# stanfordnlp/mac-network

Measured on NVIDIA H100. Metric: mac_reasoning_steps_per_sec, higher is better.
Workload: dtype bf16

## Files before the change

mac_network_b200/csrc/read_step.cuh:

```cuda
#pragma once
#include "tc_gemm.cuh"

namespace mac {

constexpr int RS_D = 512;
constexpr int RS_BM = 64;
constexpr int RS_KB = RS_D / TC_BK;
constexpr int RS_BLK = RS_BM * TC_BK * 2;
constexpr int RS_A_BYTES = RS_KB * RS_BLK;
constexpr int RS_B_HALF = 256 * TC_BK * 2;
constexpr int RS_CONSUMERS = 256;
constexpr int RS_THREADS = RS_CONSUMERS + 32;

constexpr int RS128_BM = 128;
constexpr int RS128_BLK = RS128_BM * TC_BK * 2;
constexpr int RS128_A_BYTES = RS_KB * RS128_BLK;
constexpr int RS128_STAGE = RS_B_HALF;
constexpr int RS128_STAGES = 3;
constexpr int RS128_Q0 = RS_KB;
constexpr int RS128_G1B = RS128_Q0 + 2;
constexpr int RS128_Q1 = RS128_G1B + RS_KB;
constexpr int RS128_G2A = RS128_Q1 + 2;
constexpr int RS128_G2B = RS128_G2A + RS_KB;
constexpr int RS128_SLOTS = RS128_G2B + RS_KB;
constexpr int RS128_CONSUMERS = 256;
constexpr int RS128_THREADS = RS128_CONSUMERS + 128;
constexpr int RS128_SMEM_BYTES = RS128_A_BYTES + RS128_STAGES * RS128_STAGE + 1024  +
                                 8 * (RS_KB + 2 * RS128_STAGES) ;
static_assert(RS128_SMEM_BYTES <= 232448, "over the sm_90 per-block shared memory opt-in limit");
static_assert(RS128_BLK % 1024 == 0 && RS128_STAGE % 1024 == 0 && (RS128_BM / 2) * 128 % 1024 == 0,
              "swizzled operands need 1024-byte alignment");
static_assert(2 * RS128_BLK == RS128_STAGE, "a ring slot holds two Q blocks");
constexpr int RS128_PRODUCER_REGS = 40;
constexpr int RS128_CONSUMER_REGS = 232;
static_assert(RS128_PRODUCER_REGS + 2 * RS128_CONSUMER_REGS <= 3 * (65536 / RS128_THREADS / 8 * 8), "register budget");

__device__ __forceinline__ float bf16lo(uint32_t w) { return __uint_as_float(w << 16); }
__device__ __forceinline__ float bf16hi(uint32_t w) { return __uint_as_float(w & 0xffff0000u); }

__device__ __forceinline__ void wgmma_bf16_n256(float (&d)[128], uint64_t adesc, uint64_t bdesc, uint32_t accum) {
  asm volatile(
      "{\n\t.reg .pred p;\n\t"
      "setp.ne.b32 p, %130, 0;\n\t"
      "wgmma.mma_async.sync.aligned.m64n256k16.f32.bf16.bf16 "
      "{%0, %1, %2, %3, %4, %5, %6, %7, %8, %9, %10, %11, %12, %13, %14, %15, %16, %17, %18, %19, %20, %21, %22, %23, %24, %25, %26, %27, %28, %29, %30, %31, %32, %33, %34, %35, %36, %37, %38, %39, %40, %41, %42, %43, %44, %45, %46, %47, %48, %49, %50, %51, %52, %53, %54, %55, %56, %57, %58, %59, %60, %61, %62, %63, %64, %65, %66, %67, %68, %69, %70, %71, %72, %73, %74, %75, %76, %77, %78, %79, %80, %81, %82, %83, %84, %85, %86, %87, %88, %89, %90, %91, %92, %93, %94, %95, %96, %97, %98, %99, %100, %101, %102, %103, %104, %105, %106, %107, %108, %109, %110, %111, %112, %113, %114, %115, %116, %117, %118, %119, %120, %121, %122, %123, %124, %125, %126, %127}, %128, %129, p, 1, 1, 0, 0;\n\t}"
      : "+f"(d[0]), "+f"(d[1]), "+f"(d[2]), "+f"(d[3]), "+f"(d[4]), "+f"(d[5]), "+f"(d[6]), "+f"(d[7]), "+f"(d[8]), "+f"(d[9]), "+f"(d[10]), "+f"(d[11]), "+f"(d[12]), "+f"(d[13]), "+f"(d[14]), "+f"(d[15]), "+f"(d[16]), "+f"(d[17]), "+f"(d[18]), "+f"(d[19]), "+f"(d[20]), "+f"(d[21]), "+f"(d[22]), "+f"(d[23]), "+f"(d[24]), "+f"(d[25]), "+f"(d[26]), "+f"(d[27]), "+f"(d[28]), "+f"(d[29]), "+f"(d[30]), "+f"(d[31]), "+f"(d[32]), "+f"(d[33]), "+f"(d[34]), "+f"(d[35]), "+f"(d[36]), "+f"(d[37]), "+f"(d[38]), "+f"(d[39]), "+f"(d[40]), "+f"(d[41]), "+f"(d[42]), "+f"(d[43]), "+f"(d[44]), "+f"(d[45]), "+f"(d[46]), "+f"(d[47]), "+f"(d[48]), "+f"(d[49]), "+f"(d[50]), "+f"(d[51]), "+f"(d[52]), "+f"(d[53]), "+f"(d[54]), "+f"(d[55]), "+f"(d[56]), "+f"(d[57]), "+f"(d[58]), "+f"(d[59]), "+f"(d[60]), "+f"(d[61]), "+f"(d[62]), "+f"(d[63]), "+f"(d[64]), "+f"(d[65]), "+f"(d[66]), "+f"(d[67]), "+f"(d[68]), "+f"(d[69]), "+f"(d[70]), "+f"(d[71]), "+f"(d[72]), "+f"(d[73]), "+f"(d[74]), "+f"(d[75]), "+f"(d[76]), "+f"(d[77]), "+f"(d[78]), "+f"(d[79]), "+f"(d[80]), "+f"(d[81]), "+f"(d[82]), "+f"(d[83]), "+f"(d[84]), "+f"(d[85]), "+f"(d[86]), "+f"(d[87]), "+f"(d[88]), "+f"(d[89]), "+f"(d[90]), "+f"(d[91]), "+f"(d[92]), "+f"(d[93]), "+f"(d[94]), "+f"(d[95]), "+f"(d[96]), "+f"(d[97]), "+f"(d[98]), "+f"(d[99]), "+f"(d[100]), "+f"(d[101]), "+f"(d[102]), "+f"(d[103]), "+f"(d[104]), "+f"(d[105]), "+f"(d[106]), "+f"(d[107]), "+f"(d[108]), "+f"(d[109]), "+f"(d[110]), "+f"(d[111]), "+f"(d[112]), "+f"(d[113]), "+f"(d[114]), "+f"(d[115]), "+f"(d[116]), "+f"(d[117]), "+f"(d[118]), "+f"(d[119]), "+f"(d[120]), "+f"(d[121]), "+f"(d[122]), "+f"(d[123]), "+f"(d[124]), "+f"(d[125]), "+f"(d[126]), "+f"(d[127])
      : "l"(adesc), "l"(bdesc), "r"(accum));
}
inline bool read_step_supported(int B, int N, int d) {
  return d == RS_D && N >= 1 && N <= 256 && B >= 1 && B < (1 << 22);
}

struct ReadStepParams {
  int M, N;
  const float* y;
  const float* ctrl;
  const float* bm2;
  const float* wr;
  float* logits;
};

__device__ __forceinline__ void rs_consumer_bar() { asm volatile("bar.sync 1, %0;" ::"n"(RS_CONSUMERS) : "memory"); }

__device__ __forceinline__ void rs128_wg_bar(int g) { asm volatile("bar.sync %0, 128;" ::"r"(1 + g) : "memory"); }

__device__ __forceinline__ void rs128_gemm_half(float (&acc)[128], uint32_t a_u, uint32_t ring_u, uint64_t* full,
                                                uint64_t* empty, int t0, int lane) {
  for (int j = 0; j < RS_KB; ++j) {
    const int t = t0 + j, s = t % RS128_STAGES;
    mbar_wait(&full[s], (t / RS128_STAGES) & 1);
    const uint64_t adesc = make_sw128_kmajor_desc(a_u + j * RS128_BLK);
    const uint64_t bdesc = make_sw128_kmajor_desc(ring_u + s * RS128_STAGE);
    wgmma_fence();
#pragma unroll
    for (int k = 0; k < TC_BK / 16; ++k) wgmma_bf16_n256(acc, adesc + 2 * k, bdesc + 2 * k, (j || k) ? 1u : 0u);
    wgmma_commit();
    wgmma_wait<1>();
    wgmma_hold(acc);
    if (j && lane == 0) mbar_arrive(&empty[(t - 1) % RS128_STAGES]);
  }
  wgmma_wait<0>();
  wgmma_hold(acc);
  if (lane == 0) mbar_arrive(&empty[(t0 + RS_KB - 1) % RS128_STAGES]);
}

__device__ __forceinline__ int rs128_sw_off(int r, int n, int blk) {
  return (n >> 6) * blk + r * 128 + ((((n & 63) >> 3) ^ (r & 7)) << 4) + (n & 7) * 2;
}

__global__ void __launch_bounds__(RS128_THREADS, 1)
read_step_kernel(const __grid_constant__ CUtensorMap map_p, const __grid_constant__ CUtensorMap map_q,
                 const __grid_constant__ CUtensorMap map_w1, const __grid_constant__ CUtensorMap map_w2,
                 const ReadStepParams p) {
  extern __shared__ unsigned char smem_dyn[];
  const uint32_t base_u32 = smem_u32(smem_dyn);
  unsigned char* a_tile = smem_dyn + ((1024u - (base_u32 & 1023u)) & 1023u);
  unsigned char* ring = a_tile + RS128_A_BYTES;
  uint64_t* pfull = reinterpret_cast<uint64_t*>(ring + RS128_STAGES * RS128_STAGE);
  uint64_t* full = pfull + RS_KB;
  uint64_t* empty = full + RS128_STAGES;

  const int warp = threadIdx.x >> 5, lane = threadIdx.x & 31;
  const int row0 = blockIdx.x * RS128_BM;

  if (threadIdx.x == RS128_CONSUMERS) {
    tma_prefetch_desc(&map_p);
    tma_prefetch_desc(&map_q);
    tma_prefetch_desc(&map_w1);
    tma_prefetch_desc(&map_w2);
    for (int i = 0; i < RS_KB; ++i) mbar_init(&pfull[i], 1);
    for (int i = 0; i < RS128_STAGES; ++i) {
      mbar_init(&full[i], 1);
      mbar_init(&empty[i], RS128_CONSUMERS / 32);
    }
    fence_mbar_init();
  }
  __syncthreads();

  if (warp >= RS128_CONSUMERS / 32) {
    asm volatile("setmaxnreg.dec.sync.aligned.u32 %0;" ::"n"(RS128_PRODUCER_REGS));
    if (warp == RS128_CONSUMERS / 32 && elect_one()) {
      auto load_p = [&](int j) {
        mbar_expect_tx(&pfull[j], RS128_BLK);
        tma_load_2d(a_tile + j * RS128_BLK, &map_p, j * TC_BK, row0, &pfull[j]);
      };
      for (int t = 0; t < RS128_SLOTS; ++t) {
        if (t < RS128_STAGES) load_p(t);
        else if (t == RS128_STAGES)
          for (int j = RS128_STAGES; j < RS_KB; ++j) load_p(j);
        const int s = t % RS128_STAGES;
        mbar_wait(&empty[s], ((t / RS128_STAGES) & 1) ^ 1);
        unsigned char* dst = ring + s * RS128_STAGE;
        mbar_expect_tx(&full[s], RS128_STAGE);
        if (t < RS128_G2A) {
          const int half = t >= RS128_G1B, u = t - half * RS128_G1B;
          if (u < RS_KB) {
            tma_load_2d(dst, &map_w1, u * TC_BK, 256 * half, &full[s]);
          } else {
            const int kb = 4 * half + 2 * (u - RS_KB);
            tma_load_2d(dst, &map_q, kb * TC_BK, row0, &full[s]);
            tma_load_2d(dst + RS128_BLK, &map_q, (kb + 1) * TC_BK, row0, &full[s]);
          }
        } else {
          const int half = t >= RS128_G2B, u = t - (half ? RS128_G2B : RS128_G2A);
          tma_load_2d(dst, &map_w2, u * TC_BK, 256 * half, &full[s]);
        }
      }
    }
    return;
  }

  asm volatile("setmaxnreg.inc.sync.aligned.u32 %0;" ::"n"(RS128_CONSUMER_REGS));
  const int g = warp >> 2;
  const int wt = threadIdx.x & 127;
  const int rl = 16 * (warp & 3) + (lane >> 2);
  const int cq = 2 * (lane & 3);
  const int rowg = row0 + 64 * g;
  unsigned char* a_wg = a_tile + g * (RS128_BM / 2) * 128;
  const uint32_t a_u = smem_u32(a_wg), ring_u = smem_u32(ring);
  const int prow = wt >> 3;
  const int poff = prow * 128 + (wt & 7) * 16;
  const int pcol = ((wt & 7) ^ (prow & 7)) << 3;
  int yoff[4];
#pragma unroll
  for (int u = 0; u < 4; ++u) yoff[u] = min(rowg + prow + 16 * u, p.M - 1) / p.N * RS_D + pcol;

  float acc[128];
  float4 y0[4], y1[4];
  auto load_y = [&](int j) {
#pragma unroll
    for (int u = 0; u < 4; ++u) {
      y0[u] = *reinterpret_cast<const float4*>(p.y + yoff[u] + j * TC_BK);
      y1[u] = *reinterpret_cast<const float4*>(p.y + yoff[u] + j * TC_BK + 4);
    }
  };
  load_y(0);
  for (int j = 0; j < RS_KB; ++j) {
    const int s = j % RS128_STAGES;
    mbar_wait(&pfull[j], 0);
#pragma unroll
    for (int u = 0; u < 4; ++u) {
      uint4* c = reinterpret_cast<uint4*>(a_wg + j * RS128_BLK + poff + u * 16 * 128);
      const uint4 v = *c;
      *c = make_uint4(pack_bf16(bf16lo(v.x) * y0[u].x, bf16hi(v.x) * y0[u].y), pack_bf16(bf16lo(v.y) * y0[u].z, bf16hi(v.y) * y0[u].w),
                      pack_bf16(bf16lo(v.z) * y1[u].x, bf16hi(v.z) * y1[u].y), pack_bf16(bf16lo(v.w) * y1[u].z, bf16hi(v.w) * y1[u].w));
    }
    fence_proxy_async();
    rs128_wg_bar(g);
    mbar_wait(&full[s], (j / RS128_STAGES) & 1);
    const uint64_t adesc = make_sw128_kmajor_desc(a_u + j * RS128_BLK);
    const uint64_t bdesc = make_sw128_kmajor_desc(ring_u + s * RS128_STAGE);
    wgmma_fence();
#pragma unroll
    for (int k = 0; k < TC_BK / 16; ++k) wgmma_bf16_n256(acc, adesc + 2 * k, bdesc + 2 * k, (j || k) ? 1u : 0u);
    wgmma_commit();
    if (j + 1 < RS_KB) load_y(j + 1);
    wgmma_wait<1>();
    wgmma_hold(acc);
    if (j && lane == 0) mbar_arrive(&empty[(j - 1) % RS128_STAGES]);
  }
  wgmma_wait<0>();
  wgmma_hold(acc);
  if (lane == 0) mbar_arrive(&empty[(RS_KB - 1) % RS128_STAGES]);

  uint32_t h0[64];
#pragma unroll
  for (int q = 0; q < 2; ++q) {
    const int t = RS128_Q0 + q, s = t % RS128_STAGES;
    mbar_wait(&full[s], (t / RS128_STAGES) & 1);
    const unsigned char* q_tile = ring + s * RS128_STAGE + g * (RS128_BM / 2) * 128 - 2 * q * RS128_BLK;
#pragma unroll
    for (int h = 0; h < 2; ++h) {
      const int r = rl + 8 * h;
      const bool live = rowg + r < p.M;
#pragma unroll
      for (int j = 16 * q; j < 16 * q + 16; ++j) {
        const uint32_t qv = *reinterpret_cast<const uint32_t*>(q_tile + rs128_sw_off(r, cq + 8 * j, RS128_BLK));
        h0[2 * j + h] = live ? pack_bf16(elu_fast(acc[4 * j + 2 * h] + bf16lo(qv)), elu_fast(acc[4 * j + 2 * h + 1] + bf16hi(qv)))
                             : 0u;
      }
    }
    __syncwarp();
    if (lane == 0) mbar_arrive(&empty[s]);
  }

  rs128_gemm_half(acc, a_u, ring_u, full, empty, RS128_G1B, lane);

  rs128_wg_bar(g);
#pragma unroll
  for (int h = 0; h < 2; ++h) {
    const int r = rl + 8 * h;
#pragma unroll
    for (int j = 0; j < 32; ++j) *reinterpret_cast<uint32_t*>(a_wg + rs128_sw_off(r, cq + 8 * j, RS128_BLK)) = h0[2 * j + h];
  }
#pragma unroll
  for (int q = 0; q < 2; ++q) {
    const int t = RS128_Q1 + q, s = t % RS128_STAGES;
    mbar_wait(&full[s], (t / RS128_STAGES) & 1);
    const unsigned char* q_tile = ring + s * RS128_STAGE + g * (RS128_BM / 2) * 128 - 2 * q * RS128_BLK;
#pragma unroll
    for (int h = 0; h < 2; ++h) {
      const int r = rl + 8 * h;
      const bool live = rowg + r < p.M;
#pragma unroll
      for (int j = 16 * q; j < 16 * q + 16; ++j) {
        const int n = cq + 8 * j;
        const uint32_t qv = *reinterpret_cast<const uint32_t*>(q_tile + rs128_sw_off(r, n, RS128_BLK));
        *reinterpret_cast<uint32_t*>(a_wg + rs128_sw_off(r, 256 + n, RS128_BLK)) =
            live ? pack_bf16(elu_fast(acc[4 * j + 2 * h] + bf16lo(qv)), elu_fast(acc[4 * j + 2 * h + 1] + bf16hi(qv))) : 0u;
      }
    }
    __syncwarp();
    if (lane == 0) mbar_arrive(&empty[s]);
  }
  fence_proxy_async();
  rs128_wg_bar(g);

  float part[2][2];
#pragma unroll
  for (int half = 0; half < 2; ++half) {
    rs128_gemm_half(acc, a_u, ring_u, full, empty, half ? RS128_G2B : RS128_G2A, lane);
#pragma unroll
    for (int h = 0; h < 2; ++h) {
      const int row = rowg + rl + 8 * h;
      const float* crow = p.ctrl + (size_t)(min(row, p.M - 1) / p.N) * RS_D + 256 * half;
      const float* bm2 = p.bm2 + 256 * half;
      const float* wr = p.wr + 256 * half;
      float s = 0.f;
#pragma unroll
      for (int j = 0; j < 32; ++j) {
        const int n = cq + 8 * j;
        const float2 cc = __ldg(reinterpret_cast<const float2*>(crow + n));
        const float2 bb = __ldg(reinterpret_cast<const float2*>(bm2 + n));
        const float2 ww = __ldg(reinterpret_cast<const float2*>(wr + n));
        const float t0 = elu_fast((acc[4 * j + 2 * h] + bb.x) * cc.x);
        const float t1 = elu_fast((acc[4 * j + 2 * h + 1] + bb.y) * cc.y);
        s = fmaf(t0, ww.x, s);
        s = fmaf(t1, ww.y, s);
      }
      s += __shfl_xor_sync(0xffffffffu, s, 1);
      s += __shfl_xor_sync(0xffffffffu, s, 2);
      part[half][h] = s;
    }
  }
#pragma unroll
  for (int h = 0; h < 2; ++h) {
    const int row = rowg + rl + 8 * h;
    if ((lane & 3) == 0 && row < p.M) p.logits[row] = part[0][h] + part[1][h];
  }
}

inline int read_step_launch(const void* P, const void* Q, float* logits, const void* kb_bf16, const float* y,
                            const float* control, const mac_read_weights* w, float* att, float* info, int B, int N, int d,
                            cudaStream_t stream) {
  const int M = B * N;
  CUtensorMap mp, mq, mw1, mw2;
  int st = make_tmap_2d(&mp, P, 1, (uint64_t)M, (uint64_t)d, (uint64_t)d * 2, RS128_BM, TC_BK, 1);
  if (st != MAC_OK) return st;
  st = make_tmap_2d(&mq, Q, 1, (uint64_t)M, (uint64_t)d, (uint64_t)d * 2, RS128_BM, TC_BK, 1);
  if (st != MAC_OK) return st;
  st = make_tmap_2d(&mw1, w->Wm_bf16, 1, (uint64_t)d, (uint64_t)d, (uint64_t)2 * d * 2, 256, TC_BK, 1);
  if (st != MAC_OK) return st;
  st = make_tmap_2d(&mw2, w->Wm2_bf16, 1, (uint64_t)d, (uint64_t)d, (uint64_t)d * 2, 256, TC_BK, 1);
  if (st != MAC_OK) return st;
  ReadStepParams p{};
  p.M = M; p.N = N; p.y = y; p.ctrl = control; p.bm2 = w->bm2; p.wr = w->wr; p.logits = logits;
  MAC_CUDA_TRY(cudaFuncSetAttribute(read_step_kernel, cudaFuncAttributeMaxDynamicSharedMemorySize, RS128_SMEM_BYTES));
  read_step_kernel<<<(M + RS128_BM - 1) / RS128_BM, RS128_THREADS, RS128_SMEM_BYTES, stream>>>(mp, mq, mw1, mw2, p);
  MAC_LAUNCH_CHECK();
  return mac_kb_attend_fwd(logits, 1, w->br, kb_bf16, 1, att, info, B, N, d, stream);
}

}
```

Baseline: 21560.

## Feed GEMM1 A operand from registers via ldmatrix and stream P with weights

GEMM 1 no longer loads P fully into shared memory, scales it by y in place and issues an SS wgmma. P tiles are now streamed through a two-stage ring alongside the W1 tiles, loaded into registers with ldmatrix, scaled by y in registers, and fed to register-sourced wgmma. This removes the shared-memory write-back, the async-proxy fence and the warpgroup barrier on each k-block. Q is loaded directly into the A tile, so the h epilogue updates it in place instead of staging it through the ring and a 64-register h0 buffer. The trade-off is higher register pressure from the A fragments and y values, plus a more complex barrier layout.

```diff
diff --git a/mac_network_b200/csrc/read_step.cuh b/mac_network_b200/csrc/read_step.cuh
--- a/mac_network_b200/csrc/read_step.cuh
+++ b/mac_network_b200/csrc/read_step.cuh
@@ -17,20 +17,21 @@
 constexpr int RS128_A_BYTES = RS_KB * RS128_BLK;
 constexpr int RS128_STAGE = RS_B_HALF;
 constexpr int RS128_STAGES = 3;
-constexpr int RS128_Q0 = RS_KB;
-constexpr int RS128_G1B = RS128_Q0 + 2;
-constexpr int RS128_Q1 = RS128_G1B + RS_KB;
-constexpr int RS128_G2A = RS128_Q1 + 2;
-constexpr int RS128_G2B = RS128_G2A + RS_KB;
-constexpr int RS128_SLOTS = RS128_G2B + RS_KB;
+constexpr int RS128_RING_BYTES = RS128_STAGES * RS128_STAGE;
 constexpr int RS128_CONSUMERS = 256;
 constexpr int RS128_THREADS = RS128_CONSUMERS + 128;
-constexpr int RS128_SMEM_BYTES = RS128_A_BYTES + RS128_STAGES * RS128_STAGE + 1024  +
+constexpr int RS128_SMEM_BYTES = RS128_A_BYTES + RS128_RING_BYTES + 1024  +
                                  8 * (RS_KB + 2 * RS128_STAGES) ;
 static_assert(RS128_SMEM_BYTES <= 232448, "over the sm_90 per-block shared memory opt-in limit");
 static_assert(RS128_BLK % 1024 == 0 && RS128_STAGE % 1024 == 0 && (RS128_BM / 2) * 128 % 1024 == 0,
               "swizzled operands need 1024-byte alignment");
-static_assert(2 * RS128_BLK == RS128_STAGE, "a ring slot holds two Q blocks");
+constexpr int RS128_P_STAGE = RS_B_HALF + RS128_BLK;
+constexpr int RS128_P_STAGES = 2;
+constexpr int RS128_G1_SLOTS = 2 * RS_KB;
+static_assert(RS128_P_STAGES * RS128_P_STAGE <= RS128_RING_BYTES && RS128_P_STAGE % 1024 == 0, "GEMM 1 ring");
+constexpr int RS128_STEP_SMEM_BYTES = RS128_A_BYTES + RS128_RING_BYTES + 1024  +
+                                      8 * (RS_KB + 2 * RS128_P_STAGES + 2 * RS128_STAGES) ;
+static_assert(RS128_STEP_SMEM_BYTES <= 232448, "over the sm_90 per-block shared memory opt-in limit");
 constexpr int RS128_PRODUCER_REGS = 40;
 constexpr int RS128_CONSUMER_REGS = 232;
 static_assert(RS128_PRODUCER_REGS + 2 * RS128_CONSUMER_REGS <= 3 * (65536 / RS128_THREADS / 8 * 8), "register budget");
@@ -47,6 +48,19 @@
       : "+f"(d[0]), "+f"(d[1]), "+f"(d[2]), "+f"(d[3]), "+f"(d[4]), "+f"(d[5]), "+f"(d[6]), "+f"(d[7]), "+f"(d[8]), "+f"(d[9]), "+f"(d[10]), "+f"(d[11]), "+f"(d[12]), "+f"(d[13]), "+f"(d[14]), "+f"(d[15]), "+f"(d[16]), "+f"(d[17]), "+f"(d[18]), "+f"(d[19]), "+f"(d[20]), "+f"(d[21]), "+f"(d[22]), "+f"(d[23]), "+f"(d[24]), "+f"(d[25]), "+f"(d[26]), "+f"(d[27]), "+f"(d[28]), "+f"(d[29]), "+f"(d[30]), "+f"(d[31]), "+f"(d[32]), "+f"(d[33]), "+f"(d[34]), "+f"(d[35]), "+f"(d[36]), "+f"(d[37]), "+f"(d[38]), "+f"(d[39]), "+f"(d[40]), "+f"(d[41]), "+f"(d[42]), "+f"(d[43]), "+f"(d[44]), "+f"(d[45]), "+f"(d[46]), "+f"(d[47]), "+f"(d[48]), "+f"(d[49]), "+f"(d[50]), "+f"(d[51]), "+f"(d[52]), "+f"(d[53]), "+f"(d[54]), "+f"(d[55]), "+f"(d[56]), "+f"(d[57]), "+f"(d[58]), "+f"(d[59]), "+f"(d[60]), "+f"(d[61]), "+f"(d[62]), "+f"(d[63]), "+f"(d[64]), "+f"(d[65]), "+f"(d[66]), "+f"(d[67]), "+f"(d[68]), "+f"(d[69]), "+f"(d[70]), "+f"(d[71]), "+f"(d[72]), "+f"(d[73]), "+f"(d[74]), "+f"(d[75]), "+f"(d[76]), "+f"(d[77]), "+f"(d[78]), "+f"(d[79]), "+f"(d[80]), "+f"(d[81]), "+f"(d[82]), "+f"(d[83]), "+f"(d[84]), "+f"(d[85]), "+f"(d[86]), "+f"(d[87]), "+f"(d[88]), "+f"(d[89]), "+f"(d[90]), "+f"(d[91]), "+f"(d[92]), "+f"(d[93]), "+f"(d[94]), "+f"(d[95]), "+f"(d[96]), "+f"(d[97]), "+f"(d[98]), "+f"(d[99]), "+f"(d[100]), "+f"(d[101]), "+f"(d[102]), "+f"(d[103]), "+f"(d[104]), "+f"(d[105]), "+f"(d[106]), "+f"(d[107]), "+f"(d[108]), "+f"(d[109]), "+f"(d[110]), "+f"(d[111]), "+f"(d[112]), "+f"(d[113]), "+f"(d[114]), "+f"(d[115]), "+f"(d[116]), "+f"(d[117]), "+f"(d[118]), "+f"(d[119]), "+f"(d[120]), "+f"(d[121]), "+f"(d[122]), "+f"(d[123]), "+f"(d[124]), "+f"(d[125]), "+f"(d[126]), "+f"(d[127])
       : "l"(adesc), "l"(bdesc), "r"(accum));
 }
+__device__ __forceinline__ void wgmma_bf16_n256_rs(float (&d)[128], const uint32_t (&a)[4], uint64_t bdesc, uint32_t accum) {
+  asm volatile(
+      "{\n\t.reg .pred p;\n\t"
+      "setp.ne.b32 p, %133, 0;\n\t"
+      "wgmma.mma_async.sync.aligned.m64n256k16.f32.bf16.bf16 "
+      "{%0, %1, %2, %3, %4, %5, %6, %7, %8, %9, %10, %11, %12, %13, %14, %15, %16, %17, %18, %19, %20, %21, %22, %23, %24, %25, %26, %27, %28, %29, %30, %31, %32, %33, %34, %35, %36, %37, %38, %39, %40, %41, %42, %43, %44, %45, %46, %47, %48, %49, %50, %51, %52, %53, %54, %55, %56, %57, %58, %59, %60, %61, %62, %63, %64, %65, %66, %67, %68, %69, %70, %71, %72, %73, %74, %75, %76, %77, %78, %79, %80, %81, %82, %83, %84, %85, %86, %87, %88, %89, %90, %91, %92, %93, %94, %95, %96, %97, %98, %99, %100, %101, %102, %103, %104, %105, %106, %107, %108, %109, %110, %111, %112, %113, %114, %115, %116, %117, %118, %119, %120, %121, %122, %123, %124, %125, %126, %127}, {%128, %129, %130, %131}, %132, p, 1, 1, 0;\n\t}"
+      : "+f"(d[0]), "+f"(d[1]), "+f"(d[2]), "+f"(d[3]), "+f"(d[4]), "+f"(d[5]), "+f"(d[6]), "+f"(d[7]), "+f"(d[8]), "+f"(d[9]), "+f"(d[10]), "+f"(d[11]), "+f"(d[12]), "+f"(d[13]), "+f"(d[14]), "+f"(d[15]), "+f"(d[16]), "+f"(d[17]), "+f"(d[18]), "+f"(d[19]), "+f"(d[20]), "+f"(d[21]), "+f"(d[22]), "+f"(d[23]), "+f"(d[24]), "+f"(d[25]), "+f"(d[26]), "+f"(d[27]), "+f"(d[28]), "+f"(d[29]), "+f"(d[30]), "+f"(d[31]), "+f"(d[32]), "+f"(d[33]), "+f"(d[34]), "+f"(d[35]), "+f"(d[36]), "+f"(d[37]), "+f"(d[38]), "+f"(d[39]), "+f"(d[40]), "+f"(d[41]), "+f"(d[42]), "+f"(d[43]), "+f"(d[44]), "+f"(d[45]), "+f"(d[46]), "+f"(d[47]), "+f"(d[48]), "+f"(d[49]), "+f"(d[50]), "+f"(d[51]), "+f"(d[52]), "+f"(d[53]), "+f"(d[54]), "+f"(d[55]), "+f"(d[56]), "+f"(d[57]), "+f"(d[58]), "+f"(d[59]), "+f"(d[60]), "+f"(d[61]), "+f"(d[62]), "+f"(d[63]), "+f"(d[64]), "+f"(d[65]), "+f"(d[66]), "+f"(d[67]), "+f"(d[68]), "+f"(d[69]), "+f"(d[70]), "+f"(d[71]), "+f"(d[72]), "+f"(d[73]), "+f"(d[74]), "+f"(d[75]), "+f"(d[76]), "+f"(d[77]), "+f"(d[78]), "+f"(d[79]), "+f"(d[80]), "+f"(d[81]), "+f"(d[82]), "+f"(d[83]), "+f"(d[84]), "+f"(d[85]), "+f"(d[86]), "+f"(d[87]), "+f"(d[88]), "+f"(d[89]), "+f"(d[90]), "+f"(d[91]), "+f"(d[92]), "+f"(d[93]), "+f"(d[94]), "+f"(d[95]), "+f"(d[96]), "+f"(d[97]), "+f"(d[98]), "+f"(d[99]), "+f"(d[100]), "+f"(d[101]), "+f"(d[102]), "+f"(d[103]), "+f"(d[104]), "+f"(d[105]), "+f"(d[106]), "+f"(d[107]), "+f"(d[108]), "+f"(d[109]), "+f"(d[110]), "+f"(d[111]), "+f"(d[112]), "+f"(d[113]), "+f"(d[114]), "+f"(d[115]), "+f"(d[116]), "+f"(d[117]), "+f"(d[118]), "+f"(d[119]), "+f"(d[120]), "+f"(d[121]), "+f"(d[122]), "+f"(d[123]), "+f"(d[124]), "+f"(d[125]), "+f"(d[126]), "+f"(d[127])
+      : "r"(a[0]), "r"(a[1]), "r"(a[2]), "r"(a[3]), "l"(bdesc), "r"(accum));
+}
+__device__ __forceinline__ void ldmatrix_x4(uint32_t (&r)[4], uint32_t addr) {
+  asm volatile("ldmatrix.sync.aligned.m8n8.x4.shared.b16 {%0, %1, %2, %3}, [%4];"
+               : "=r"(r[0]), "=r"(r[1]), "=r"(r[2]), "=r"(r[3]) : "r"(addr) : "memory");
+}
 inline bool read_step_supported(int B, int N, int d) {
   return d == RS_D && N >= 1 && N <= 256 && B >= 1 && B < (1 << 22);
 }
@@ -96,8 +110,10 @@
   const uint32_t base_u32 = smem_u32(smem_dyn);
   unsigned char* a_tile = smem_dyn + ((1024u - (base_u32 & 1023u)) & 1023u);
   unsigned char* ring = a_tile + RS128_A_BYTES;
-  uint64_t* pfull = reinterpret_cast<uint64_t*>(ring + RS128_STAGES * RS128_STAGE);
-  uint64_t* full = pfull + RS_KB;
+  uint64_t* qfull = reinterpret_cast<uint64_t*>(ring + RS128_RING_BYTES);
+  uint64_t* pfull = qfull + RS_KB;
+  uint64_t* pempty = pfull + RS128_P_STAGES;
+  uint64_t* full = pempty + RS128_P_STAGES;
   uint64_t* empty = full + RS128_STAGES;
 
   const int warp = threadIdx.x >> 5, lane = threadIdx.x & 31;
@@ -108,7 +124,11 @@
     tma_prefetch_desc(&map_q);
     tma_prefetch_desc(&map_w1);
     tma_prefetch_desc(&map_w2);
-    for (int i = 0; i < RS_KB; ++i) mbar_init(&pfull[i], 1);
+    for (int i = 0; i < RS_KB; ++i) mbar_init(&qfull[i], 1);
+    for (int i = 0; i < RS128_P_STAGES; ++i) {
+      mbar_init(&pfull[i], 1);
+      mbar_init(&pempty[i], RS128_CONSUMERS / 32);
+    }
     for (int i = 0; i < RS128_STAGES; ++i) {
       mbar_init(&full[i], 1);
       mbar_init(&empty[i], RS128_CONSUMERS / 32);
@@ -120,31 +140,28 @@
   if (warp >= RS128_CONSUMERS / 32) {
     asm volatile("setmaxnreg.dec.sync.aligned.u32 %0;" ::"n"(RS128_PRODUCER_REGS));
     if (warp == RS128_CONSUMERS / 32 && elect_one()) {
-      auto load_p = [&](int j) {
-        mbar_expect_tx(&pfull[j], RS128_BLK);
-        tma_load_2d(a_tile + j * RS128_BLK, &map_p, j * TC_BK, row0, &pfull[j]);
+      auto load_q = [&](int j) {
+        mbar_expect_tx(&qfull[j], RS128_BLK);
+        tma_load_2d(a_tile + j * RS128_BLK, &map_q, j * TC_BK, row0, &qfull[j]);
       };
-      for (int t = 0; t < RS128_SLOTS; ++t) {
-        if (t < RS128_STAGES) load_p(t);
-        else if (t == RS128_STAGES)
-          for (int j = RS128_STAGES; j < RS_KB; ++j) load_p(j);
+      for (int t = 0; t < RS128_G1_SLOTS; ++t) {
+        if (t == RS128_P_STAGES)
+          for (int j = 0; j < RS_KB / 2; ++j) load_q(j);
+        else if (t == RS_KB)
+          for (int j = RS_KB / 2; j < RS_KB; ++j) load_q(j);
+        const int s = t % RS128_P_STAGES, u = t % RS_KB;
+        mbar_wait(&pempty[s], ((t / RS128_P_STAGES) & 1) ^ 1);
+        unsigned char* dst = ring + s * RS128_P_STAGE;
+        mbar_expect_tx(&pfull[s], RS128_P_STAGE);
+        tma_load_2d(dst, &map_w1, u * TC_BK, 256 * (t / RS_KB), &pfull[s]);
+        tma_load_2d(dst + RS_B_HALF, &map_p, u * TC_BK, row0, &pfull[s]);
+      }
+      for (int s = 0; s < RS128_P_STAGES; ++s) mbar_wait(&pempty[s], ((RS128_G1_SLOTS / RS128_P_STAGES) & 1) ^ 1);
+      for (int t = 0; t < 2 * RS_KB; ++t) {
         const int s = t % RS128_STAGES;
         mbar_wait(&empty[s], ((t / RS128_STAGES) & 1) ^ 1);
-        unsigned char* dst = ring + s * RS128_STAGE;
         mbar_expect_tx(&full[s], RS128_STAGE);
-        if (t < RS128_G2A) {
-          const int half = t >= RS128_G1B, u = t - half * RS128_G1B;
-          if (u < RS_KB) {
-            tma_load_2d(dst, &map_w1, u * TC_BK, 256 * half, &full[s]);
-          } else {
-            const int kb = 4 * half + 2 * (u - RS_KB);
-            tma_load_2d(dst, &map_q, kb * TC_BK, row0, &full[s]);
-            tma_load_2d(dst + RS128_BLK, &map_q, (kb + 1) * TC_BK, row0, &full[s]);
-          }
-        } else {
-          const int half = t >= RS128_G2B, u = t - (half ? RS128_G2B : RS128_G2A);
-          tma_load_2d(dst, &map_w2, u * TC_BK, 256 * half, &full[s]);
-        }
+        tma_load_2d(ring + s * RS128_STAGE, &map_w2, (t % RS_KB) * TC_BK, 256 * (t / RS_KB), &full[s]);
       }
     }
     return;
@@ -152,114 +169,88 @@
 
   asm volatile("setmaxnreg.inc.sync.aligned.u32 %0;" ::"n"(RS128_CONSUMER_REGS));
   const int g = warp >> 2;
-  const int wt = threadIdx.x & 127;
   const int rl = 16 * (warp & 3) + (lane >> 2);
   const int cq = 2 * (lane & 3);
   const int rowg = row0 + 64 * g;
   unsigned char* a_wg = a_tile + g * (RS128_BM / 2) * 128;
   const uint32_t a_u = smem_u32(a_wg), ring_u = smem_u32(ring);
-  const int prow = wt >> 3;
-  const int poff = prow * 128 + (wt & 7) * 16;
-  const int pcol = ((wt & 7) ^ (prow & 7)) << 3;
-  int yoff[4];
-#pragma unroll
-  for (int u = 0; u < 4; ++u) yoff[u] = min(rowg + prow + 16 * u, p.M - 1) / p.N * RS_D + pcol;
+  const int lrow = 64 * g + 16 * (warp & 3) + (lane & 15);
+  const uint32_t p_u = ring_u + RS_B_HALF + lrow * 128;
+  const int lsw = lrow & 7, lch = lane >> 4;
+  int yoff[2];
+#pragma unroll
+  for (int h = 0; h < 2; ++h) yoff[h] = min(rowg + rl + 8 * h, p.M - 1) / p.N * RS_D + cq;
+  float2 yv[4][2][2];
+  auto load_y = [&](int j) {
+#pragma unroll
+    for (int k = 0; k < 4; ++k)
+#pragma unroll
+      for (int h = 0; h < 2; ++h)
+#pragma unroll
+        for (int e = 0; e < 2; ++e) yv[k][h][e] = *reinterpret_cast<const float2*>(p.y + yoff[h] + j * TC_BK + 16 * k + 8 * e);
+  };
 
   float acc[128];
-  float4 y0[4], y1[4];
-  auto load_y = [&](int j) {
-#pragma unroll
-    for (int u = 0; u < 4; ++u) {
-      y0[u] = *reinterpret_cast<const float4*>(p.y + yoff[u] + j * TC_BK);
-      y1[u] = *reinterpret_cast<const float4*>(p.y + yoff[u] + j * TC_BK + 4);
-    }
+  uint32_t afrag[2][4][4];
+  auto gemm1_half = [&](int half) {
+#pragma unroll
+    for (int j = 0; j < RS_KB; ++j) {
+      const int t = half * RS_KB + j, s = t % RS128_P_STAGES;
+      uint32_t(&f)[4][4] = afrag[j & 1];
+      mbar_wait(&pfull[s], (t / RS128_P_STAGES) & 1);
+#pragma unroll
+      for (int k = 0; k < 4; ++k) ldmatrix_x4(f[k], p_u + s * RS128_P_STAGE + (((2 * k + lch) ^ lsw) << 4));
+#pragma unroll
+      for (int k = 0; k < 4; ++k)
+#pragma unroll
+        for (int i = 0; i < 4; ++i) {
+          const float2 yy = yv[k][i & 1][i >> 1];
+          f[k][i] = pack_bf16(bf16lo(f[k][i]) * yy.x, bf16hi(f[k][i]) * yy.y);
+        }
+      const uint64_t bdesc = make_sw128_kmajor_desc(ring_u + s * RS128_P_STAGE);
+      wgmma_fence();
+#pragma unroll
+      for (int k = 0; k < TC_BK / 16; ++k) wgmma_bf16_n256_rs(acc, f[k], bdesc + 2 * k, (j || k) ? 1u : 0u);
+      wgmma_commit();
+      if (half == 0 || j + 1 < RS_KB) load_y((j + 1) % RS_KB);
+      wgmma_wait<1>();
+      wgmma_hold(acc);
+      if (j && lane == 0) mbar_arrive(&pempty[(t - 1) % RS128_P_STAGES]);
+    }
+    wgmma_wait<0>();
+    wgmma_hold(acc);
+    if (lane == 0) mbar_arrive(&pempty[(half * RS_KB + RS_KB - 1) % RS128_P_STAGES]);
   };
+  auto h_epilogue = [&](int half) {
+#pragma unroll
+    for (int q = 0; q < 4; ++q) {
+      mbar_wait(&qfull[4 * half + q], 0);
+#pragma unroll
+      for (int h = 0; h < 2; ++h) {
+        const int r = rl + 8 * h;
+        const bool live = rowg + r < p.M;
+#pragma unroll
+        for (int j = 8 * q; j < 8 * q + 8; ++j) {
+          uint32_t* c = reinterpret_cast<uint32_t*>(a_wg + rs128_sw_off(r, 256 * half + cq + 8 * j, RS128_BLK));
+          const uint32_t qv = *c;
+          *c = live ? pack_bf16(elu_fast(acc[4 * j + 2 * h] + bf16lo(qv)), elu_fast(acc[4 * j + 2 * h + 1] + bf16hi(qv))) : 0u;
+        }
+      }
+    }
+  };
+
   load_y(0);
-  for (int j = 0; j < RS_KB; ++j) {
-    const int s = j % RS128_STAGES;
-    mbar_wait(&pfull[j], 0);
-#pragma unroll
-    for (int u = 0; u < 4; ++u) {
-      uint4* c = reinterpret_cast<uint4*>(a_wg + j * RS128_BLK + poff + u * 16 * 128);
-      const uint4 v = *c;
-      *c = make_uint4(pack_bf16(bf16lo(v.x) * y0[u].x, bf16hi(v.x) * y0[u].y), pack_bf16(bf16lo(v.y) * y0[u].z, bf16hi(v.y) * y0[u].w),
-                      pack_bf16(bf16lo(v.z) * y1[u].x, bf16hi(v.z) * y1[u].y), pack_bf16(bf16lo(v.w) * y1[u].z, bf16hi(v.w) * y1[u].w));
-    }
-    fence_proxy_async();
-    rs128_wg_bar(g);
-    mbar_wait(&full[s], (j / RS128_STAGES) & 1);
-    const uint64_t adesc = make_sw128_kmajor_desc(a_u + j * RS128_BLK);
-    const uint64_t bdesc = make_sw128_kmajor_desc(ring_u + s * RS128_STAGE);
-    wgmma_fence();
-#pragma unroll
-    for (int k = 0; k < TC_BK / 16; ++k) wgmma_bf16_n256(acc, adesc + 2 * k, bdesc + 2 * k, (j || k) ? 1u : 0u);
-    wgmma_commit();
-    if (j + 1 < RS_KB) load_y(j + 1);
-    wgmma_wait<1>();
-    wgmma_hold(acc);
-    if (j && lane == 0) mbar_arrive(&empty[(j - 1) % RS128_STAGES]);
-  }
-  wgmma_wait<0>();
-  wgmma_hold(acc);
-  if (lane == 0) mbar_arrive(&empty[(RS_KB - 1) % RS128_STAGES]);
-
-  uint32_t h0[64];
-#pragma unroll
-  for (int q = 0; q < 2; ++q) {
-    const int t = RS128_Q0 + q, s = t % RS128_STAGES;
-    mbar_wait(&full[s], (t / RS128_STAGES) & 1);
-    const unsigned char* q_tile = ring + s * RS128_STAGE + g * (RS128_BM / 2) * 128 - 2 * q * RS128_BLK;
-#pragma unroll
-    for (int h = 0; h < 2; ++h) {
-      const int r = rl + 8 * h;
-      const bool live = rowg + r < p.M;
-#pragma unroll
-      for (int j = 16 * q; j < 16 * q + 16; ++j) {
-        const uint32_t qv = *reinterpret_cast<const uint32_t*>(q_tile + rs128_sw_off(r, cq + 8 * j, RS128_BLK));
-        h0[2 * j + h] = live ? pack_bf16(elu_fast(acc[4 * j + 2 * h] + bf16lo(qv)), elu_fast(acc[4 * j + 2 * h + 1] + bf16hi(qv)))
-                             : 0u;
-      }
-    }
-    __syncwarp();
-    if (lane == 0) mbar_arrive(&empty[s]);
-  }
-
-  rs128_gemm_half(acc, a_u, ring_u, full, empty, RS128_G1B, lane);
-
-  rs128_wg_bar(g);
-#pragma unroll
-  for (int h = 0; h < 2; ++h) {
-    const int r = rl + 8 * h;
-#pragma unroll
-    for (int j = 0; j < 32; ++j) *reinterpret_cast<uint32_t*>(a_wg + rs128_sw_off(r, cq + 8 * j, RS128_BLK)) = h0[2 * j + h];
-  }
-#pragma unroll
-  for (int q = 0; q < 2; ++q) {
-    const int t = RS128_Q1 + q, s = t % RS128_STAGES;
-    mbar_wait(&full[s], (t / RS128_STAGES) & 1);
-    const unsigned char* q_tile = ring + s * RS128_STAGE + g * (RS128_BM / 2) * 128 - 2 * q * RS128_BLK;
-#pragma unroll
-    for (int h = 0; h < 2; ++h) {
-      const int r = rl + 8 * h;
-      const bool live = rowg + r < p.M;
-#pragma unroll
-      for (int j = 16 * q; j < 16 * q + 16; ++j) {
-        const int n = cq + 8 * j;
-        const uint32_t qv = *reinterpret_cast<const uint32_t*>(q_tile + rs128_sw_off(r, n, RS128_BLK));
-        *reinterpret_cast<uint32_t*>(a_wg + rs128_sw_off(r, 256 + n, RS128_BLK)) =
-            live ? pack_bf16(elu_fast(acc[4 * j + 2 * h] + bf16lo(qv)), elu_fast(acc[4 * j + 2 * h + 1] + bf16hi(qv))) : 0u;
-      }
-    }
-    __syncwarp();
-    if (lane == 0) mbar_arrive(&empty[s]);
-  }
+  gemm1_half(0);
+  h_epilogue(0);
+  gemm1_half(1);
+  h_epilogue(1);
   fence_proxy_async();
   rs128_wg_bar(g);
 
   float part[2][2];
 #pragma unroll
   for (int half = 0; half < 2; ++half) {
-    rs128_gemm_half(acc, a_u, ring_u, full, empty, half ? RS128_G2B : RS128_G2A, lane);
+    rs128_gemm_half(acc, a_u, ring_u, full, empty, half * RS_KB, lane);
 #pragma unroll
     for (int h = 0; h < 2; ++h) {
       const int row = rowg + rl + 8 * h;
@@ -305,8 +296,8 @@
   if (st != MAC_OK) return st;
   ReadStepParams p{};
   p.M = M; p.N = N; p.y = y; p.ctrl = control; p.bm2 = w->bm2; p.wr = w->wr; p.logits = logits;
-  MAC_CUDA_TRY(cudaFuncSetAttribute(read_step_kernel, cudaFuncAttributeMaxDynamicSharedMemorySize, RS128_SMEM_BYTES));
-  read_step_kernel<<<(M + RS128_BM - 1) / RS128_BM, RS128_THREADS, RS128_SMEM_BYTES, stream>>>(mp, mq, mw1, mw2, p);
+  MAC_CUDA_TRY(cudaFuncSetAttribute(read_step_kernel, cudaFuncAttributeMaxDynamicSharedMemorySize, RS128_STEP_SMEM_BYTES));
+  read_step_kernel<<<(M + RS128_BM - 1) / RS128_BM, RS128_THREADS, RS128_STEP_SMEM_BYTES, stream>>>(mp, mq, mw1, mw2, p);
   MAC_LAUNCH_CHECK();
   return mac_kb_attend_fwd(logits, 1, w->br, kb_bf16, 1, att, info, B, N, d, stream);
 }
diff --git a/profiles/read_step_rs.py b/profiles/read_step_rs.py
--- /dev/null
+++ b/profiles/read_step_rs.py
@@ -0,0 +1,61 @@
+import argparse
+import json
+import os
+import shutil
+import sys
+import tempfile
+
+import numpy as np
+
+sys.path.insert(0, os.path.dirname(os.path.dirname(os.path.abspath(__file__))))
+from profiles.read_step_128 import LIB_REL, ROOT, SIDES, bench, device_info, spread, tree_copy
+
+
+def main():
+    ap = argparse.ArgumentParser()
+    ap.add_argument("out_dir")
+    ap.add_argument("--base-lib", required=True)
+    ap.add_argument("--runs", type=int, default=3)
+    ap.add_argument("--roof-runs", type=int, default=6)
+    args = ap.parse_args()
+    out = {"device": device_info(), "runs": args.runs, "roof_runs": args.roof_runs,
+           "headline_args": "--gpus 1 --steps 480 --warmup 12 --skip-cpu"}
+    tmp = tempfile.mkdtemp(prefix="read_step_rs_")
+    try:
+        trees = {"base": tree_copy(os.path.join(tmp, "base"), os.path.abspath(args.base_lib)),
+                 "new": tree_copy(os.path.join(tmp, "new"), os.path.join(ROOT, LIB_REL))}
+        dumps = {s: os.path.join(tmp, "dump_" + s) for s in SIDES}
+
+        roof = {s: [] for s in SIDES}
+        for _ in range(args.roof_runs):
+            for s in SIDES:
+                roof[s].append(bench(trees[s], ["--rooflines-only"])["read_step_fused"]["us"])
+        out["read_step_fused_us"] = {s: spread(roof[s]) for s in SIDES}
+        out["read_step_fused_speedup"] = out["read_step_fused_us"]["base"]["median"] / out["read_step_fused_us"]["new"]["median"]
+
+        lines = {s: {"headline": [], "bf16_gqa": []} for s in SIDES}
+        for i in range(args.runs):
+            for s in SIDES:
+                extra = ["--gpus", "1", "--steps", "480", "--warmup", "12", "--skip-cpu"]
+                line = bench(trees[s], extra + (["--dump-outputs", dumps[s]] if i == 0 else []))
+                lines[s]["headline"].append(line["value"])
+                lines[s]["bf16_gqa"].append(line["sub_lines"]["bf16_gqa"]["value"])
+        out["reasoning_steps_per_s"] = {s: {k: spread(v) for k, v in lines[s].items()} for s in SIDES}
+        out["headline_speedup"] = (out["reasoning_steps_per_s"]["new"]["headline"]["median"] /
+                                   out["reasoning_steps_per_s"]["base"]["headline"]["median"])
+
+        same = {}
+        for name in sorted(os.listdir(dumps["base"])):
+            a, b = np.load(os.path.join(dumps["base"], name)), np.load(os.path.join(dumps["new"], name))
+            same[name] = bool(a.shape == b.shape and a.dtype == b.dtype and a.tobytes() == b.tobytes())
+        out["outputs_bit_identical"] = same
+    finally:
+        shutil.rmtree(tmp, ignore_errors=True)
+    os.makedirs(args.out_dir, exist_ok=True)
+    with open(os.path.join(args.out_dir, "read_step_rs_h100.json"), "w") as f:
+        json.dump(out, f, indent=1)
+    print(json.dumps(out))
+
+
+if __name__ == "__main__":
+    main()
```

Measured after the change: 19460 (median of 6 runs). 9.7% lower.
